# pengzai6666/deequ

Hardware: AMD Instinct MI355X
Metric: rows/sec & HBM GB/s for analyzer-suite scan, 1B rows x 8 cols, 1/2/4/8 GPUs (higher is better)
Workload: dtype int64+f64; 1 GPU; C2: 1000000000 rows/GPU x 8 cols (4 int64 + 4 fp64), 65 scan-shareable analyzers (incl. 8 ApproxCountDistinct) fused in one pass; rows_per_gpu=1000000000, columns=8, analyzers=65, parallelism=dp1 (row shards, states all-gathered over RCCL)

## Files before the change

### deequ_amd/_lib.py

```python
from __future__ import annotations

import ctypes
import os
from ctypes import (POINTER, Structure, c_char_p, c_double, c_int, c_int32, c_int64, c_size_t,
                    c_uint8, c_uint64, c_void_p)

LIB_PATH = os.environ.get("DEEQU_AMD_LIB") or os.path.join(
    os.path.dirname(os.path.abspath(__file__)), "libdeequ_amd.so")

DQ_OK, DQ_ERR_INVALID, DQ_ERR_UNSUPPORTED, DQ_ERR_DEVICE, DQ_ERR_OOM, DQ_ERR_STATE, DQ_ERR_SPACE = range(7)

DQ_T_BOOL, DQ_T_INT8, DQ_T_INT16, DQ_T_INT32, DQ_T_INT64, DQ_T_FLOAT32, DQ_T_FLOAT64, DQ_T_UTF8 = range(1, 9)
DQ_T_DECIMAL128 = 9
DQ_COL_DEVICE = 0x1

(DQ_OP_SIZE, DQ_OP_COMPLETENESS, DQ_OP_COMPLIANCE, DQ_OP_SUM, DQ_OP_MEAN, DQ_OP_STDDEV,
 DQ_OP_MINIMUM, DQ_OP_MAXIMUM, DQ_OP_APPROX_COUNT_DISTINCT, DQ_OP_DATATYPE, DQ_OP_MIN_LENGTH,
 DQ_OP_MAX_LENGTH, DQ_OP_CORRELATION, DQ_OP_PATTERN_MATCH) = range(1, 15)

DQ_P_COLUMN, DQ_P_LIT_INT, DQ_P_LIT_FLOAT, DQ_P_LIT_NULL, DQ_P_COALESCE, DQ_P_LIT_STRING = 1, 2, 3, 4, 5, 6
DQ_P_CAST_DOUBLE = 7
DQ_P_CAST = 8
DQ_P_EQ, DQ_P_NE, DQ_P_LT, DQ_P_LE, DQ_P_GT, DQ_P_GE, DQ_P_EQ_NULLSAFE = 10, 11, 12, 13, 14, 15, 16
DQ_P_IS_NULL, DQ_P_IS_NOT_NULL = 20, 21
# ... 150 lines not shown
    "dq_diag_key_pack": (c_int, [c_char_p, c_int32, POINTER(c_uint64), c_char_p, POINTER(c_int32), POINTER(c_int32)]),
    "dq_diag_uuid_pack": (c_int, [c_char_p, c_int32, POINTER(c_uint64), c_char_p, POINTER(c_int32)]),
    "dq_diag_eval_predicate": (c_int, [POINTER(DqPredicate), POINTER(DqColumn), c_int, c_int64, c_void_p]),
    "dq_diag_regex_match": (c_int, [c_char_p, c_int32, c_char_p, c_int64, POINTER(c_int32), POINTER(c_int32),
                                    POINTER(c_int32)]),
    "dq_diag_regex_match_mode": (c_int, [c_char_p, c_int32, c_int32, c_char_p, c_int64, POINTER(c_int32),
                                         POINTER(c_int32), POINTER(c_int32), c_void_p, c_int64, POINTER(c_int64)]),
    "dq_diag_plan_match_tasks": (c_int, [c_void_p, POINTER(c_int32), POINTER(c_int32)]),
    "dq_diag_kll_sketch": (c_int, [c_void_p, c_void_p, c_int64, c_int32, c_double, c_int64, c_void_p, c_int64,
                                   POINTER(c_int64)]),
    "dq_diag_schema_cell": (c_int, [c_int32, c_char_p, c_int64, c_int32, c_int32, POINTER(c_int32),
                                    POINTER(c_int64)]),
    "dq_diag_decimal_to_double": (c_int, [c_uint64, c_int64, c_int32, POINTER(c_double), POINTER(c_int32)]),
    "dq_diag_decimal_bytes": (c_int, [c_uint64, c_int64, c_char_p, POINTER(c_int32)]),
    "dq_diag_plan_groups": (c_int, [c_void_p, POINTER(c_int64), c_int32, POINTER(c_int32), POINTER(c_int64)]),
}


SIGNATURES = {
    "dq_last_error": (c_char_p, []),
    "dq_abi_version": (c_int, []),
    "dq_device_count": (c_int, [POINTER(c_int)]),
    "dq_release_cached_memory": (c_int, [c_int]),
    "dq_ctx_create": (c_int, [c_int, c_int, POINTER(c_void_p)]),
    "dq_ctx_destroy": (c_int, [c_void_p]),
    "dq_plan_create": (c_int, [c_void_p, POINTER(DqOp), c_int, POINTER(c_int32), c_int, POINTER(c_void_p)]),
    "dq_plan_destroy": (c_int, [c_void_p]),
    "dq_plan_create_packed": (c_int, [c_void_p, c_char_p, c_size_t, POINTER(c_int32), c_int, POINTER(c_void_p)]),
    "dq_op_supported": (c_int, [POINTER(DqOp), POINTER(c_int32), c_int]),
    "dq_plan_consume": (c_int, [c_void_p, POINTER(DqColumn), c_int, c_int64]),
# ... 130 lines not shown
PLAN_LAUNCHES = ("regex", "string_pass", "hll", "datatype", "strlen", "corr", "dec")


def diag_plan_groups(plan_handle):
    n = ctypes.c_int32(0)
    launches = (c_int64 * 10)()
    check(lib().dq_diag_plan_groups(plan_handle, None, 0, ctypes.byref(n), launches))
    groups = (c_int64 * (6 * max(1, n.value)))()
    check(lib().dq_diag_plan_groups(plan_handle, groups, n.value, ctypes.byref(n), launches))
    out = [tuple(groups[6 * g:6 * g + 6]) for g in range(n.value)]
    info = dict(zip(PLAN_LAUNCHES, launches[:7]))
    info.update(rows=launches[7], dec_per_cu=launches[8], n_cu=launches[9])
    return out, info


REGEX_MODES = {"find_non_empty": 0, "find": 1, "full": 2}


def diag_regex_match(pattern: bytes, text: bytes, mode: str = "find_non_empty", want_image: bool = False):
    m, ns, nc = c_int32(0), c_int32(0), c_int32(0)
    size = c_int64(0)
    args = (pattern, len(pattern), REGEX_MODES[mode], text, len(text), ctypes.byref(m), ctypes.byref(ns), ctypes.byref(nc))
    check(lib().dq_diag_regex_match_mode(*args, None, 0, ctypes.byref(size)))
    if not want_image:
        return m.value, ns.value, nc.value
    buf = ctypes.create_string_buffer(size.value)
    check(lib().dq_diag_regex_match_mode(*args, buf, size.value, ctypes.byref(size)))
    return m.value, ns.value, nc.value, buf.raw


# ... 28 lines not shown
```

### deequ_amd/csrc/dq_api.cpp

```cpp
#include <algorithm>
#include <cmath>
#include <cstdio>
#include <cstdlib>
#include <cstring>
#include <deque>
#include <limits>
#include <memory>
#include <mutex>
#include <unordered_map>
#include <string>
#include <vector>

#include "dq_internal.h"
#include "dq_keypack.h"
#include "dq_uuidpack.h"
#include "dq_numparse.h"
#include "dq_decimal.h"
#include "dq_predeval.h"
#include "dq_regex.h"
#include "dq_kll.h"
#include "dq_quantile.h"
#include "dq_schema.h"
#include "../../include/deequ_amd_diag.h"
#include "hll_p9_tables.h"
// ... 822 lines not shown
  DevBuf d_tasks, d_groups, d_ranges, d_hll, d_progs, d_insns, d_pool, d_acc, d_partials, d_regs,
      d_cols, d_masks, d_mask_words, d_dtype, d_dtype_counts, d_len, d_len_out, d_corr, d_corr_part, d_corr_acc, d_str, d_rx, d_rx_dfas, d_rx_out,
      d_dec, d_dec_acc, d_dec_part, d_match, d_match_words;
  int64_t mask_words = 0;
  void* h_desc = nullptr;
  size_t h_desc_size = 0;
  void* h_back = nullptr;
  size_t h_back_size = 0;
  hipEvent_t desc_done = nullptr;
  bool desc_pending = false;
  int64_t total_rows = 0;
  int target_blocks = 2048;
  int n_cu = 0;
  int scan_rounds = 6;
  int max_blocks = 0;
  std::vector<int64_t> diag_group_bpt;
  int64_t diag_launch_bpt[7] = {0, 0, 0, 0, 0, 0, 0};
  int64_t diag_rows = 0;
  int64_t cap_blocks(int64_t bpt) const { return max_blocks > 0 ? std::min<int64_t>(bpt, max_blocks) : bpt; }
  uint64_t batch_seq = 0;
  hipEvent_t copy_done[2] = {nullptr, nullptr}, scan_done[2] = {nullptr, nullptr};
  hipStream_t side_stream = nullptr;
  hipEvent_t side_ready = nullptr, side_done = nullptr;

  ~dq_plan() {
    if (stream) {
      (void)hipStreamSynchronize(stream);
    }
    if (side_stream) (void)hipStreamSynchronize(side_stream);
    if (side_ready) (void)hipEventDestroy(side_ready);
// ... 453 lines not shown
                      std::max<size_t>(1, plan->scan_tasks.size()) * sizeof(PartRange);
  if (e == hipSuccess) e = PinnedPool::get().alloc(plan->h_desc_size, &plan->h_desc);
  if (e != hipSuccess) {
    delete plan;
    return fail(DQ_ERR_DEVICE, std::string("stream/event/pinned allocation failed: ") + hipGetErrorString(e));
  }
  plan->resize_stage(n_columns);
  hipDeviceProp_t prop;
  if (hipGetDeviceProperties(&prop, ctx->device) == hipSuccess)
  {
    plan->target_blocks = std::max(256, prop.multiProcessorCount * 8);
    plan->n_cu = prop.multiProcessorCount;
  }
  if (const char* r = std::getenv("DQ_SCAN_ROUNDS")) plan->scan_rounds = std::max(0, std::atoi(r));
  if (const char* r = std::getenv("DQ_SCAN_MAX_BLOCKS")) plan->max_blocks = std::max(0, std::atoi(r));
  if ((s = dq_plan_reset(plan)) != DQ_OK) {
    delete plan;
    return s;
  }
  *out = plan;
  return DQ_OK;
}

extern "C" dq_status dq_plan_destroy(dq_plan* plan) {
  delete plan;
  return DQ_OK;
}

extern "C" dq_status dq_diag_plan_groups(dq_plan* plan, int64_t* groups, int32_t capacity, int32_t* n_groups,
                                         int64_t* launches) {
// ... 3 lines not shown
  const bool ran = plan->diag_group_bpt.size() == plan->groups.size() && plan->diag_rows > 0;
  for (size_t g = 0; g < plan->groups.size() && (int32_t)g < capacity; ++g) {
    const ScanGroup& G = plan->groups[g];
    int64_t* o = groups + 6 * g;
    o[0] = G.kind;
    o[1] = G.kind == 0 ? 0 : G.ptype;
    o[2] = G.np;
    o[3] = (int64_t)G.tasks.size();
    o[4] = ran ? plan->diag_group_bpt[g] : 0;
    o[5] = plan->group_per_cu.size() == plan->groups.size() ? plan->group_per_cu[g] : 0;
  }
  for (int k = 0; k < 7; ++k) launches[k] = ran ? plan->diag_launch_bpt[k] : 0;
  launches[7] = ran ? plan->diag_rows : 0;
  launches[8] = plan->dec_per_cu > 0 ? plan->dec_per_cu : 0;
  launches[9] = plan->n_cu;
  return DQ_OK;
}

extern "C" void* dq_plan_stream(dq_plan* plan) { return plan ? (void*)plan->stream : nullptr; }

extern "C" dq_status dq_plan_op_status(dq_plan* plan, int op) {
  if (!plan) return fail(DQ_ERR_INVALID, "plan is NULL");
  if (op < 0 || op >= (int)plan->slots.size()) return fail(DQ_ERR_INVALID, "op index out of range");
  if (plan->op_status.size() != plan->slots.size()) return fail(DQ_ERR_STATE, "dq_plan_finish has not run");
  if (plan->op_status[op] != DQ_OK && op < (int)plan->op_message.size() && !plan->op_message[op].empty())
    return fail(plan->op_status[op], plan->op_message[op]);
  if (plan->op_status[op] != DQ_OK)
    return fail(plan->op_status[op], "a string -> double cast in this op's predicate met a number off the exact "
                                     "fast path (> 19 significant digits, |exponent| > 22 or hex): route it to Spark");
  return DQ_OK;
// ... 197 lines not shown
                                                                 plan->groups[q].np);
      }
      const int per_cu = plan->group_per_cu[g];
      if (per_cu > 0) bpt = std::max<int64_t>(1, (int64_t)plan->n_cu * per_cu * plan->scan_rounds / ng);
    }
    bpt = plan->cap_blocks(std::max<int64_t>(1, std::min<int64_t>(bpt, chunks)));
    bpt = std::max<int64_t>(bpt, (chunks + (((int64_t)1 << 27) / kScanRowAlign) - 1) /
                                     (((int64_t)1 << 27) / kScanRowAlign));
    group_bpt[g] = bpt;
    group_base[g] = part_total;
    for (int64_t i = 0; i < ng; ++i)
      h_ranges[plan->groups[g].tasks[i]] = PartRange{part_total + i * bpt, (int32_t)bpt, 0};
    part_total += bpt * ng;
  }
  plan->diag_group_bpt = group_bpt;
  for (int64_t& b : plan->diag_launch_bpt) b = 0;
  plan->diag_rows = n_rows;
  if (n_scan > 0) DQ_TRY(plan->d_partials.ensure((size_t)part_total * sizeof(ScanAcc)));

  DQ_HIP(hipMemcpyAsync(plan->d_cols.ptr, h_cols, n_columns * sizeof(DevColumn), hipMemcpyHostToDevice, plan->stream));
  if (n_progs > 0)
    DQ_HIP(hipMemcpyAsync(plan->d_masks.ptr, h_masks, n_progs * sizeof(DevMask), hipMemcpyHostToDevice, plan->stream));
  if (n_scan > 0)
    DQ_HIP(hipMemcpyAsync(plan->d_ranges.ptr, h_ranges, n_scan * sizeof(PartRange), hipMemcpyHostToDevice, plan->stream));
  DQ_HIP(hipEventRecord(plan->desc_done, plan->stream));
  plan->desc_pending = true;

  const DevColumn* d_cols = static_cast<const DevColumn*>(plan->d_cols.ptr);
  const DevMask* d_masks = static_cast<const DevMask*>(plan->d_masks.ptr);
  const int n_match = (int)plan->match_tasks.size();
// ... 32 lines not shown
    hipStream_t ss = side ? plan->side_stream : plan->stream;
    int64_t bpt = std::max<int64_t>(1, plan->target_blocks / n_str);
    bpt = plan->cap_blocks(std::min<int64_t>(bpt, chunks));
    plan->diag_launch_bpt[1] = bpt;
    DQ_HIP(launch_string_pass(static_cast<const StrTask*>(plan->d_str.ptr), n_str, d_cols, d_masks, n_rows, (int)bpt,
                              static_cast<uint32_t*>(plan->d_regs.ptr),
                              static_cast<unsigned long long*>(plan->d_dtype_counts.ptr), ss));
    if (side) DQ_HIP(hipEventRecord(plan->side_done, ss));
  }
  if (n_scan > 0) {
    ScanAcc* parts = static_cast<ScanAcc*>(plan->d_partials.ptr);
    const ScanTask* d_tasks = static_cast<const ScanTask*>(plan->d_tasks.ptr);
    const int32_t* d_groups = static_cast<const int32_t*>(plan->d_groups.ptr);
    for (size_t g = 0; g < plan->groups.size(); ++g) {
      const ScanGroup& G = plan->groups[g];
      if (G.kind == 2)
        DQ_HIP(launch_scan_fast(G.ptype, G.np, d_tasks, d_groups + G.dev_offset, (int)G.tasks.size(), d_cols, n_rows,
                                (int)group_bpt[g], parts + group_base[g], static_cast<uint32_t*>(plan->d_regs.ptr),
                                plan->stream));
      else
        DQ_HIP(launch_scan_group(G.kind, G.ptype, G.np, d_tasks, d_groups + G.dev_offset, (int)G.tasks.size(),
                                 d_cols, d_masks, n_rows, (int)group_bpt[g], parts + group_base[g],
                                 static_cast<uint32_t*>(plan->d_regs.ptr), plan->stream));
    }
    DQ_HIP(launch_scan_reduce(parts, static_cast<const PartRange*>(plan->d_ranges.ptr), n_scan,
                              static_cast<ScanAcc*>(plan->d_acc.ptr), plan->stream));
  }
  const int n_hll = (int)plan->hll_launch.size();
  if (n_hll > 0) {
    int64_t bpt = std::max<int64_t>(1, plan->target_blocks / n_hll);
    bpt = plan->cap_blocks(std::min<int64_t>(bpt, chunks));
    plan->diag_launch_bpt[2] = bpt;
    DQ_HIP(launch_hll(static_cast<const HllTask*>(plan->d_hll.ptr), n_hll, d_cols, d_masks, n_rows, (int)bpt,
                      static_cast<uint32_t*>(plan->d_regs.ptr), plan->stream));
  }
// ... 948 lines not shown
```

### deequ_amd/csrc/dq_internal.h

```cpp
#pragma once

#include <hip/hip_runtime.h>
#include <stdint.h>

#include "../../include/deequ_amd.h"

namespace dq {

constexpr int kBlock = 256;
constexpr int kMaxPreds = 8;
constexpr int kMaxStack = 8;
constexpr int kHllM = 512;
constexpr int kHllIdxShift = 55;
constexpr uint64_t kHllWPadding = 1ull << 8;
constexpr int kScanRowAlign = 2048;

struct DevColumn {
  const uint8_t* validity;
  const void* values;
  const int32_t* offsets;
  int32_t type;
  int32_t pad;
};

// ... 365 lines not shown
                                  unsigned long long big_cap, uint32_t* d_smax, int write_all, hipStream_t stream,
                                  const FreqCompact* compact = nullptr);
hipError_t launch_freq_expand(const FreqTable& T, const FreqCompact& cmp, hipStream_t stream);
hipError_t launch_freq_export_compact(const FreqCompact& cmp, uint64_t n_slices, unsigned long long min_count,
                                      const FreqOut& out, const uint32_t* d_smax, hipStream_t stream);
hipError_t launch_freq_rehash(const FreqSlot* d_old, uint64_t old_n, const FreqTable& T, hipStream_t stream);

hipError_t launch_scan_group(int kind, int ptype, int np, const ScanTask* d_tasks,
                             const int32_t* d_group, int n_group, const DevColumn* d_cols,
                             const DevMask* d_masks, int64_t n_rows, int blocks_per_task,
                             ScanAcc* d_partials, uint32_t* d_hll_regs, hipStream_t stream);
constexpr int FAST_STATS = 8;
constexpr int FAST_HLL = 16;
hipError_t launch_scan_fast(int ptype, int variant, const ScanTask* d_tasks, const int32_t* d_group, int n_group,
                            const DevColumn* d_cols, int64_t n_rows, int blocks_per_task, ScanAcc* d_partials,
                            uint32_t* d_hll_regs, hipStream_t stream);
int scan_fast_blocks_per_cu(int ptype, int variant);
hipError_t launch_diag_hash(int blocks, int iters, bool with_hll, uint64_t* sink, hipStream_t s);
int scan_group_blocks_per_cu(int kind, int ptype, int np);
hipError_t launch_scan_reduce(const ScanAcc* d_partials, const PartRange* d_ranges, int n_tasks,
                              ScanAcc* d_acc, hipStream_t stream);
hipError_t launch_string_pass(const StrTask* d_tasks, int n_tasks, const DevColumn* d_cols, const DevMask* d_masks,
                              int64_t n_rows, int blocks_per_task, uint32_t* d_registers, unsigned long long* d_counts,
                              hipStream_t stream);
hipError_t launch_hll(const HllTask* d_tasks, int n_tasks, const DevColumn* d_cols,
                      const DevMask* d_masks, int64_t n_rows, int blocks_per_task,
                      uint32_t* d_registers, hipStream_t stream);
hipError_t launch_predicates(const PredProgram* d_progs, int n_progs, const PredInsn* d_insns,
                             const uint8_t* d_pool, const DevColumn* d_cols, int64_t n_rows,
                             uint64_t* d_mask_words, int64_t words_per_mask, bool with_cast, hipStream_t stream,
                             const uint64_t* d_match_words = nullptr);
hipError_t launch_match_mask(const MatchTask* d_tasks, int n_tasks, const DevColumn* d_cols, const uint8_t* d_dfas,
// ... 186 lines not shown
```

### deequ_amd/csrc/dq_scan_fast.hip

```cpp
#include "dq_scan_common.h"

namespace dq {

namespace {

enum FastPK : int { PK_NONE = 0, PK_LT_I = 1, PK_EQ_I = 2, PK_LT_F = 3, PK_EQ_F = 4 };

constexpr uint32_t kRankMarker = 0xFFFFFFFFu;

__device__ inline uint32_t sel32(uint32_t x, uint32_t m, uint32_t c) {
  uint32_t r;
  asm("v_bitop3_b32 %0, %1, %2, %3 bitop3:0xe2" : "=v"(r) : "v"(x), "v"(m), "v"(c));
  return r;
}

__device__ inline double i64_to_f64(uint32_t lo, uint32_t hi) {
  return fma((double)(int32_t)hi, 0x1p32, (double)lo);
}

__device__ inline double uniform_f64(double v) {
  const uint64_t b = __builtin_bit_cast(uint64_t, v);
  const uint32_t lo = __builtin_amdgcn_readfirstlane((uint32_t)b), hi = __builtin_amdgcn_readfirstlane((uint32_t)(b >> 32));
  return __builtin_bit_cast(double, ((uint64_t)hi << 32) | lo);
}
// ... 128 lines not shown
  }
}

typedef uint32_t v4u __attribute__((ext_vector_type(4)));

#ifndef DQ_FAST_UNROLL
#define DQ_FAST_UNROLL 4
#endif
#ifndef DQ_FAST_WAVES
#define DQ_FAST_WAVES 1
#endif
#ifndef DQ_VALID_AUX
#define DQ_VALID_AUX 0
#endif
constexpr int kFastUnroll = DQ_FAST_UNROLL;

constexpr int64_t kNtMinRows = (int64_t)1 << 24;
struct FastLoad {
  v4u vec[kFastUnroll];
  uint32_t vb[kFastUnroll];
};

__device__ inline void fast_load(FastLoad& L, __amdgpu_buffer_rsrc_t rv, __amdgpu_buffer_rsrc_t rvalid, uint32_t it,
                                 bool nt) {
  constexpr uint32_t ROWS_PER_ITER = (uint32_t)kBlock * 2 * kFastUnroll;
  const uint32_t tid = threadIdx.x;
#pragma unroll
  for (int u = 0; u < kFastUnroll; ++u) {
    const uint32_t r0 = it * ROWS_PER_ITER + ((uint32_t)u * kBlock + tid) * 2u;
    if (nt) {
// ... 99 lines not shown
    a.n_sel += bit;
    a.n_rows += 1;
    fast_row<T, PK, STATS, false, MEMBER, EXACT>(a, lo, hi, m, shift, cshift, dsum, lit_i, lit_f, lregs, false);
    if constexpr (__is_same(T, double) && STATS) {
      const double x = __builtin_bit_cast(double, ((uint64_t)hi << 32) | lo);
      if (bit && x != x) *s_nan = 1u;
    }
    if constexpr (HLL) {
      double unused = 0.0;
      fast_row<T, PK_NONE, false, true, MEMBER>(a, lo, hi, m, shift, cshift, unused, lit_i, lit_f, lregs, true);
    }
  }
  if constexpr (__is_same(T, double) && STATS) neumaier_add(a.fs, a.fc, dsum);
}

__device__ inline void fast_acc_init(FastAcc& a) {
  a.n_sel = a.n_rows = 0u;
  a.isum = 0u;
  a.s1 = a.s2 = 0.0;
  a.fs = a.fc = 0.0;
  a.fmin = __builtin_huge_val();
  a.fmax = -__builtin_huge_val();
  a.pc = 0u;
}

}

#ifdef DQ_SCAN_DIAG
__device__ unsigned long long g_scan_diag[4];
#define DQ_SCAN_COUNT(i) do { if (threadIdx.x == 0) atomicAdd(&g_scan_diag[i], 1ull); } while (0)
#else
#define DQ_SCAN_COUNT(i) do { } while (0)
#endif

template <typename T, int PK, bool STATS, bool HLL>
__global__ __launch_bounds__(kBlock) __attribute__((amdgpu_waves_per_eu(DQ_FAST_WAVES))) void dq_scan_fast_kernel(const ScanTask* __restrict__ tasks,
                                                              const int32_t* __restrict__ group,
                                                              const DevColumn* __restrict__ cols, int64_t n_rows,
                                                              ScanAcc* partials, uint32_t* __restrict__ hll_regs) {
  constexpr bool FP = __is_same(T, double);
  constexpr bool INT_STATS = !FP && STATS;
  const ScanTask& task = tasks[group[blockIdx.y]];
  int64_t row_begin, row_end;
  chunk_of_block(n_rows, row_begin, row_end);
  const bool nt = n_rows >= kNtMinRows;
  const uint32_t span = (uint32_t)(row_end - row_begin);
  __shared__ uint32_t lregs[kHllM];
  __shared__ uint32_t lflag[kHllM / 32];
  __shared__ uint32_t s_nan;
  if constexpr (HLL) {
    for (int r = threadIdx.x; r < kHllM; r += kBlock) lregs[r] = 0xFFFFFFFFu;
  }
  if (threadIdx.x == 0) s_nan = 0u;
  __syncthreads();
  const DevColumn& col = cols[task.primary];
  const __amdgpu_buffer_rsrc_t rv = make_rsrc(static_cast<const uint64_t*>(col.values) + row_begin, span * 8u);
  const bool has_valid = col.validity != nullptr;
  const uint32_t no_valid = has_valid ? 0u : 0xffu;
  const __amdgpu_buffer_rsrc_t rvalid =
      make_rsrc(has_valid ? col.validity + (row_begin >> 3) : nullptr, has_valid ? (span + 7u) >> 3 : 0u);
  int64_t lit_i = 0;
  double lit_f = 0.0;
  bool inv = false;
  if constexpr (PK != PK_NONE) {
    lit_i = task.preds[0].lit_i;
    lit_f = task.preds[0].lit_f;
    inv = (task.preds[0].cmp_sel & CS_INV) != 0;
  }

  const uint32_t lane = threadIdx.x & 63u;
  const uint32_t wave = threadIdx.x >> 6;
  uint32_t sh_lo = 0u, sh_hi = 0u;
  uint32_t any_lo = 0u, any_hi = 0u;
// ... 34 lines not shown
      member = true;
      break;
    }
  }
  sh_lo = __builtin_amdgcn_readfirstlane(sh_lo);
  sh_hi = __builtin_amdgcn_readfirstlane(sh_hi);
  const double shift = uniform_f64(FP ? __builtin_bit_cast(double, ((uint64_t)sh_hi << 32) | sh_lo)
                                      : i64_to_f64(sh_lo, sh_hi));
  const double cshift = uniform_f64(0x1.8p52 + shift);
  const double shift_any = FP ? shift : i64_to_f64(any_lo, any_hi);

  FastAcc a;
  fast_acc_init(a);
  constexpr uint32_t ROWS_PER_ITER = (uint32_t)kBlock * 2u * kFastUnroll;
  const uint32_t full_iters = span / ROWS_PER_ITER;
  if (member) {
    fast_main_loop<T, PK, STATS, HLL, true>(a, rv, rvalid, no_valid, full_iters, sh_lo, sh_hi, shift, cshift, lit_i,
                                            lit_f, lregs, &s_nan, nt);
    fast_tail<T, PK, STATS, HLL, true>(a, rv, rvalid, no_valid, full_iters * ROWS_PER_ITER, span, sh_lo, sh_hi,
                                       shift, cshift, lit_i, lit_f, lregs, &s_nan);
  } else {
    fast_main_loop<T, PK, STATS, HLL, false>(a, rv, rvalid, no_valid, full_iters, sh_lo, sh_hi, shift, cshift, lit_i,
                                             lit_f, lregs, &s_nan, nt);
    fast_tail<T, PK, STATS, HLL, false>(a, rv, rvalid, no_valid, full_iters * ROWS_PER_ITER, span, sh_lo, sh_hi,
                                        shift, cshift, lit_i, lit_f, lregs, &s_nan);
  }

  bool exact_stats = false;
  uint32_t mom_sel = a.n_sel;
  if constexpr (INT_STATS) {
    const double dmax = (a.fmin <= a.fmax) ? fmax(fabs(a.fmin), fabs(a.fmax)) : 0.0;
    const bool bad = a.n_rows > 0 && (dmax >= 0x1p50 || dmax * (double)a.n_rows >= 0x1p62 || a.s2 != a.s2);
    if (__syncthreads_or(bad)) {
      DQ_SCAN_COUNT(0);
      exact_stats = true;
      FastAcc e;
      fast_acc_init(e);
      if (found_any)
        fast_tail<T, PK_NONE, true, false, true, true>(e, rv, rvalid, no_valid, 0u, span, any_lo, any_hi, shift_any,
                                                       cshift, lit_i, lit_f, lregs, &s_nan);
      else
        fast_tail<T, PK_NONE, true, false, false, true>(e, rv, rvalid, no_valid, 0u, span, 0u, 0u, 0.0, cshift,
                                                        lit_i, lit_f, lregs, &s_nan);
      a.s1 = e.s1;
      a.s2 = e.s2;
      mom_sel = e.n_sel;
      a.fmin = e.fmin;
      a.fmax = e.fmax;
    } else {
      a.fmin = a.fmin + shift;
      a.fmax = a.fmax + shift;
      a.s1 = (double)(int64_t)(a.isum - (uint64_t)a.n_rows * (((uint64_t)sh_hi << 32) | sh_lo));
    }
  }

  const bool lane0 = lane == 0;
  double mom_shift = (INT_STATS && exact_stats) ? (found_any ? shift_any : 0.0) : shift;
  uint64_t mom_w = 0u;
  double S1 = 0.0, S2 = 0.0;
  if constexpr (STATS) {
    mom_w = wave_sum_u64(mom_sel);
    S1 = wave_sum_f64(a.s1);
    S2 = wave_sum_f64(a.s2);
    double wn = 0.0, wmean = 0.0;
    bool cancel = false;
    if (lane0 && mom_w > 0) {
      wn = (double)mom_w;
      wmean = mom_shift + S1 / wn;
      cancel = moments_cancel(wn, S1, S2);
    }
    if (__syncthreads_or(cancel)) {
      const double m = block_mean_of_waves(wn, wmean);
      if (fabs(m) < (FP ? 0x1p1000 : 0x1p62)) {
        uint32_t m_lo, m_hi;
        double m_shift;
        if constexpr (FP) {
          m_shift = m;
          const uint64_t b = __builtin_bit_cast(uint64_t, m);
// ... 50 lines not shown
        const uint32_t idx = h.hi >> 23;
        if (bit && ((lflag[idx >> 5] >> (idx & 31)) & 1u)) atomicMax(&lregs[idx], hll_rank_exact(h));
      }
      __syncthreads();
    }
    uint32_t* out = hll_regs + (int64_t)task.hll * kHllM;
    for (int r = threadIdx.x; r < kHllM; r += kBlock) {
      const uint32_t v = lregs[r];
      if (v) atomicMax(&out[r], v);
    }
  }
  __syncthreads();
  DQ_SCAN_COUNT(3);

  const uint64_t rows_w = wave_sum_u64(a.n_rows);
  const uint64_t sel_w = wave_sum_u64(a.n_sel);
  const uint64_t unsel_w = rows_w - sel_w;
  const uint64_t sh_bits = ((uint64_t)sh_hi << 32) | sh_lo;
  uint64_t isum = 0u;
  double mean = 0.0, m2 = 0.0, fs = 0.0, fc = 0.0;
  if constexpr (STATS) {
    isum = a.isum;
    fs = a.fs;
    fc = a.fc;
    if (lane0) {
      if constexpr (!FP) isum -= unsel_w * sh_bits;
      if (mom_w > 0) {
        const double n = (double)mom_w;
        mean = mom_shift + S1 / n;
        m2 = S2 - S1 * S1 / n;
        m2 = (m2 < 0.0) ? 0.0 : m2;
      }
      if constexpr (FP) {
        if (unsel_w > 0) {
          const double u = (double)unsel_w;
          const double p = u * shift;
          const double pe = (p - p == 0.0) ? fma(u, shift, -p) : 0.0;
          two_sum_merge(fs, fc, -p, -pe);
        }
      }
    }
  }
  uint64_t pm[1] = {0u}, pn[1] = {0u};
  if constexpr (PK != PK_NONE) {
    if (lane0) {
      bool pc_shift;
      if constexpr (PK == PK_LT_I) pc_shift = (int64_t)sh_bits < lit_i;
      else if constexpr (PK == PK_EQ_I) pc_shift = (int64_t)sh_bits == lit_i;
      else if constexpr (PK == PK_LT_F) pc_shift = shift < lit_f;
      else pc_shift = shift == lit_f;
      uint64_t c_all = inv ? rows_w - a.pc : a.pc;
      if (pc_shift != inv) c_all -= unsel_w;
      pm[0] = c_all;
      pn[0] = sel_w;
    }
  }
  const bool block_nan = FP && STATS && s_nan != 0u;
  block_reduce_store<1>(lane0 ? rows_w : 0u, lane0 ? rows_w : 0u, lane0 ? mom_w : 0u,
                        (threadIdx.x == 0 && block_nan) ? 1u : 0u, (int64_t)isum, INT64_MAX, INT64_MIN, fs, fc,
                        a.fmin, a.fmax, mean, m2, pm, pn, PK != PK_NONE ? 1 : 0,
                        &partials[(int64_t)blockIdx.y * gridDim.x + blockIdx.x]);
}

template <typename T, bool STATS, bool HLL>
static const void* fast_ptr(int pk) {
  switch (pk) {
    case PK_LT_I: return reinterpret_cast<const void*>(&dq_scan_fast_kernel<T, PK_LT_I, STATS, HLL>);
// ... 14 lines not shown
  return fast_ptr<T, false, false>(pk);
}

static const void* fast_kernel_for(int ptype, int variant) {
  if (ptype == DQ_T_INT64) return fast_kernel<int64_t>(variant);
  if (ptype == DQ_T_FLOAT64) {
    const int pk = variant & 7;
    if (pk == PK_LT_I || pk == PK_EQ_I) return nullptr;
    return fast_kernel<double>(variant);
  }
  return nullptr;
}

hipError_t launch_scan_fast(int ptype, int variant, const ScanTask* d_tasks, const int32_t* d_group, int n_group,
                            const DevColumn* d_cols, int64_t n_rows, int blocks_per_task, ScanAcc* d_partials,
                            uint32_t* d_hll_regs, hipStream_t stream) {
  if (n_group <= 0) return hipSuccess;
  const void* fn = fast_kernel_for(ptype, variant);
  if (!fn) return hipErrorInvalidValue;
  void* args[] = {&d_tasks, &d_group, &d_cols, &n_rows, &d_partials, &d_hll_regs};
#ifdef DQ_SCAN_DIAG
  {
    unsigned long long z[4] = {0, 0, 0, 0};
    (void)hipMemcpyToSymbolAsync(HIP_SYMBOL(g_scan_diag), z, sizeof(z), 0, hipMemcpyHostToDevice, stream);
    const hipError_t e = hipLaunchKernel(fn, dim3(blocks_per_task, n_group), dim3(kBlock), args, 0, stream);
    (void)hipMemcpyFromSymbolAsync(z, HIP_SYMBOL(g_scan_diag), sizeof(z), 0, hipMemcpyDeviceToHost, stream);
    (void)hipStreamSynchronize(stream);
    std::fprintf(stderr, "[scan_diag] rows %lld blocks %llu (x%d tasks): exact-int64 redo %llu, moment-guard redo %llu, "
                 "HLL marker re-rank %llu\n", (long long)n_rows, z[3], n_group, z[0], z[1], z[2]);
    return e;
  }
#endif
  return hipLaunchKernel(fn, dim3(blocks_per_task, n_group), dim3(kBlock), args, 0, stream);
}

// ... 10 lines not shown
```

### include/deequ_amd_diag.h

```cpp
#ifndef DEEQU_AMD_DIAG_H
#define DEEQU_AMD_DIAG_H

#include <stdint.h>
#include "deequ_amd.h"

#ifdef __cplusplus
extern "C" {
#endif

dq_status dq_diag_hash_rate(int device, int with_hll, int reps, double* hashes_per_sec);

dq_status dq_diag_freq_paths(dq_freq* f, int64_t* out);

dq_status dq_diag_freq_test_flags(dq_freq* f, int32_t flags);

dq_status dq_diag_parse_double(const uint8_t* s, int64_t n, double* out, int32_t* ok);

dq_status dq_diag_eval_predicate(const dq_predicate* p, const dq_column* columns, int n_columns, int64_t n_rows,
                                 uint8_t* out);

dq_status dq_diag_table_hash(int device, const uint64_t* k0, const uint64_t* k1, const uint32_t* len, int64_t n,
                             uint64_t* out);

dq_status dq_diag_key_pack(const uint8_t* key, int32_t len, uint64_t* packed, uint8_t* back, int32_t* back_len,
// ... 12 lines not shown

dq_status dq_diag_kll_sketch(const double* values, const uint8_t* valid, int64_t n, int32_t sketch_size,
                             double shrinking_factor, int64_t slab_rows, void* out, int64_t capacity,
                             int64_t* required);

dq_status dq_diag_schema_cell(int32_t kind, const uint8_t* text, int64_t n, int32_t precision, int32_t scale,
                              int32_t* result, int64_t* value);

dq_status dq_diag_decimal_to_double(uint64_t lo, int64_t hi, int32_t scale, double* out, int32_t* tier);

dq_status dq_diag_decimal_bytes(uint64_t lo, int64_t hi, uint8_t* out, int32_t* len);

dq_status dq_diag_plan_groups(dq_plan* plan, int64_t* groups, int32_t capacity, int32_t* n_groups,
                              int64_t* launches);

#ifdef __cplusplus
}
#endif

#endif
```

Measured before the change: 74.17 billion rows/s.

## Add lane-mask scan path using wave-level validity bitmasks for HLL groups

Adds a lane-mask variant of the fast scan kernel. Each wave loads 64-bit validity words through scalar loads, uses them as exec masks via inverse ballot, and counts selected rows with popcount, instead of having every lane load and shift validity bytes. HLL keys are batched and grouped before LDS min updates. The finish logic is adjusted for moments and predicate counts, since masked-off rows are no longer folded in as shift values. The path is on by default for HLL variants and needs 4-byte-aligned validity. It brings extra register pressure and new numeric paths for integer sums.

```diff
diff --git a/deequ_amd/_lib.py b/deequ_amd/_lib.py
--- a/deequ_amd/_lib.py
+++ b/deequ_amd/_lib.py
@@ -188,6 +188,7 @@
     "dq_diag_decimal_to_double": (c_int, [c_uint64, c_int64, c_int32, POINTER(c_double), POINTER(c_int32)]),
     "dq_diag_decimal_bytes": (c_int, [c_uint64, c_int64, c_char_p, POINTER(c_int32)]),
     "dq_diag_plan_groups": (c_int, [c_void_p, POINTER(c_int64), c_int32, POINTER(c_int32), POINTER(c_int64)]),
+    "dq_diag_plan_lanemask": (c_int, [c_void_p, POINTER(c_int32), c_int32, POINTER(c_int32)]),
 }
 
 
@@ -348,6 +349,14 @@
     return out, info
 
 
+def diag_plan_lanemask(plan_handle):
+    n = ctypes.c_int32(0)
+    check(lib().dq_diag_plan_lanemask(plan_handle, None, 0, ctypes.byref(n)))
+    tasks = (c_int32 * max(1, n.value))()
+    check(lib().dq_diag_plan_lanemask(plan_handle, tasks, n.value, ctypes.byref(n)))
+    return [bool(tasks[t]) for t in range(n.value)]
+
+
 REGEX_MODES = {"find_non_empty": 0, "find": 1, "full": 2}
 
 
diff --git a/deequ_amd/csrc/dq_api.cpp b/deequ_amd/csrc/dq_api.cpp
--- a/deequ_amd/csrc/dq_api.cpp
+++ b/deequ_amd/csrc/dq_api.cpp
@@ -860,6 +860,8 @@
   int n_cu = 0;
   int scan_rounds = 6;
   int max_blocks = 0;
+  int lanemask_mode = 1;
+  std::vector<int32_t> diag_task_lanemask;
   std::vector<int64_t> diag_group_bpt;
   int64_t diag_launch_bpt[7] = {0, 0, 0, 0, 0, 0, 0};
   int64_t diag_rows = 0;
@@ -1343,6 +1345,7 @@
   }
   if (const char* r = std::getenv("DQ_SCAN_ROUNDS")) plan->scan_rounds = std::max(0, std::atoi(r));
   if (const char* r = std::getenv("DQ_SCAN_MAX_BLOCKS")) plan->max_blocks = std::max(0, std::atoi(r));
+  if (const char* r = std::getenv("DQ_SCAN_LANEMASK")) plan->lanemask_mode = std::min(2, std::max(0, std::atoi(r)));
   if ((s = dq_plan_reset(plan)) != DQ_OK) {
     delete plan;
     return s;
@@ -1376,6 +1379,16 @@
   launches[7] = ran ? plan->diag_rows : 0;
   launches[8] = plan->dec_per_cu > 0 ? plan->dec_per_cu : 0;
   launches[9] = plan->n_cu;
+  return DQ_OK;
+}
+
+extern "C" dq_status dq_diag_plan_lanemask(dq_plan* plan, int32_t* tasks, int32_t capacity, int32_t* n_tasks) {
+  if (!plan || !n_tasks || capacity < 0 || (capacity > 0 && !tasks))
+    return fail(DQ_ERR_INVALID, "dq_diag_plan_lanemask: NULL argument");
+  *n_tasks = (int32_t)plan->scan_tasks.size();
+  const bool ran = plan->diag_task_lanemask.size() == plan->scan_tasks.size() && plan->diag_rows > 0;
+  for (size_t t = 0; t < plan->scan_tasks.size() && (int32_t)t < capacity; ++t)
+    tasks[t] = ran ? plan->diag_task_lanemask[t] : 0;
   return DQ_OK;
 }
 
@@ -1603,6 +1616,7 @@
     part_total += bpt * ng;
   }
   plan->diag_group_bpt = group_bpt;
+  plan->diag_task_lanemask.assign((size_t)n_scan, 0);
   for (int64_t& b : plan->diag_launch_bpt) b = 0;
   plan->diag_rows = n_rows;
   if (n_scan > 0) DQ_TRY(plan->d_partials.ensure((size_t)part_total * sizeof(ScanAcc)));
@@ -1665,11 +1679,14 @@
     const int32_t* d_groups = static_cast<const int32_t*>(plan->d_groups.ptr);
     for (size_t g = 0; g < plan->groups.size(); ++g) {
       const ScanGroup& G = plan->groups[g];
-      if (G.kind == 2)
+      if (G.kind == 2) {
+        const bool lanemask = scan_fast_lanemask_variant(plan->lanemask_mode, G.np);
+        for (int32_t t : G.tasks)
+          plan->diag_task_lanemask[t] = scan_fast_lanemask(lanemask, h_cols[plan->scan_tasks[t].primary].validity);
         DQ_HIP(launch_scan_fast(G.ptype, G.np, d_tasks, d_groups + G.dev_offset, (int)G.tasks.size(), d_cols, n_rows,
                                 (int)group_bpt[g], parts + group_base[g], static_cast<uint32_t*>(plan->d_regs.ptr),
-                                plan->stream));
-      else
+                                lanemask, plan->stream));
+      } else
         DQ_HIP(launch_scan_group(G.kind, G.ptype, G.np, d_tasks, d_groups + G.dev_offset, (int)G.tasks.size(),
                                  d_cols, d_masks, n_rows, (int)group_bpt[g], parts + group_base[g],
                                  static_cast<uint32_t*>(plan->d_regs.ptr), plan->stream));
diff --git a/deequ_amd/csrc/dq_internal.h b/deequ_amd/csrc/dq_internal.h
--- a/deequ_amd/csrc/dq_internal.h
+++ b/deequ_amd/csrc/dq_internal.h
@@ -403,8 +403,14 @@
 constexpr int FAST_HLL = 16;
 hipError_t launch_scan_fast(int ptype, int variant, const ScanTask* d_tasks, const int32_t* d_group, int n_group,
                             const DevColumn* d_cols, int64_t n_rows, int blocks_per_task, ScanAcc* d_partials,
-                            uint32_t* d_hll_regs, hipStream_t stream);
+                            uint32_t* d_hll_regs, bool lanemask, hipStream_t stream);
 int scan_fast_blocks_per_cu(int ptype, int variant);
+__host__ __device__ inline bool scan_fast_lanemask(bool lanemask, const uint8_t* validity) {
+  return lanemask && (reinterpret_cast<uintptr_t>(validity) & 3u) == 0u;
+}
+inline bool scan_fast_lanemask_variant(int mode, int variant) {
+  return mode >= 2 || (mode == 1 && (variant & FAST_HLL) != 0);
+}
 hipError_t launch_diag_hash(int blocks, int iters, bool with_hll, uint64_t* sink, hipStream_t s);
 int scan_group_blocks_per_cu(int kind, int ptype, int np);
 hipError_t launch_scan_reduce(const ScanAcc* d_partials, const PartRange* d_ranges, int n_tasks,
diff --git a/deequ_amd/csrc/dq_scan_fast.hip b/deequ_amd/csrc/dq_scan_fast.hip
--- a/deequ_amd/csrc/dq_scan_fast.hip
+++ b/deequ_amd/csrc/dq_scan_fast.hip
@@ -166,6 +166,10 @@
 #define DQ_VALID_AUX 0
 #endif
 constexpr int kFastUnroll = DQ_FAST_UNROLL;
+#ifndef DQ_LM_HASH_GROUP
+#define DQ_LM_HASH_GROUP 4
+#endif
+constexpr int kLmHashGroup = DQ_LM_HASH_GROUP;
 
 constexpr int64_t kNtMinRows = (int64_t)1 << 24;
 struct FastLoad {
@@ -295,6 +299,186 @@
   if constexpr (__is_same(T, double) && STATS) neumaier_add(a.fs, a.fc, dsum);
 }
 
+typedef uint32_t v2u __attribute__((ext_vector_type(2)));
+typedef uint32_t lm_words __attribute__((ext_vector_type(16), aligned(4)));
+constexpr int kLmRows = 8;
+
+struct LmLoad {
+  v2u v[kLmRows];
+};
+struct LmMasks {
+  uint64_t m[kLmRows];
+};
+
+template <int AUX>
+__device__ inline void lm_load_aux(LmLoad& L, __amdgpu_buffer_rsrc_t rv, uint32_t it) {
+  const uint32_t tid = threadIdx.x;
+  const uint32_t r0 = it * ((uint32_t)kBlock * kLmRows) + (tid >> 6) * (64u * kLmRows) + (tid & 63u);
+#pragma unroll
+  for (int u = 0; u < kLmRows; ++u)
+    L.v[u] = __builtin_amdgcn_raw_buffer_load_b64(rv, (int)((r0 + (uint32_t)u * 64u) * 8u), 0, AUX);
+}
+__device__ inline void lm_load(LmLoad& L, __amdgpu_buffer_rsrc_t rv, uint32_t it, bool nt) {
+  if (nt) lm_load_aux<2>(L, rv, it);
+  else lm_load_aux<0>(L, rv, it);
+}
+
+__device__ inline void lm_load_masks(LmMasks& M, const uint8_t* vbase, uint32_t off) {
+  if (vbase) {
+    const lm_words w = *(const __attribute__((address_space(4))) lm_words*)(vbase + off);
+#pragma unroll
+    for (int u = 0; u < kLmRows; ++u) M.m[u] = ((uint64_t)w[2 * u + 1] << 32) | w[2 * u];
+  } else {
+#pragma unroll
+    for (int u = 0; u < kLmRows; ++u) M.m[u] = ~0ull;
+  }
+}
+
+template <typename T, int PK>
+__device__ inline bool fast_pred(uint32_t lo, uint32_t hi, int64_t lit_i, double lit_f) {
+  constexpr bool INT = !__is_same(T, double);
+  if constexpr (PK == PK_LT_I) return (int64_t)(((uint64_t)hi << 32) | lo) < lit_i;
+  else if constexpr (PK == PK_EQ_I) return (int64_t)(((uint64_t)hi << 32) | lo) == lit_i;
+  else {
+    const double xd = INT ? i64_to_f64(lo, hi) : __builtin_bit_cast(double, ((uint64_t)hi << 32) | lo);
+    if constexpr (PK == PK_LT_F) return xd < lit_f;
+    else return xd == lit_f;
+  }
+}
+
+template <typename T, int PK, bool STATS, bool HLL>
+__device__ inline void lm_compute(FastAcc& a, uint32_t& sel, const LmLoad& L, const uint8_t* vbase, uint32_t voff,
+                                  double shift, double cshift, int64_t lit_i, double lit_f, uint32_t* lregs,
+                                  uint32_t* s_nan) {
+  constexpr bool FP = __is_same(T, double);
+  constexpr int G = kLmHashGroup;
+  LmMasks M;
+  lm_load_masks(M, vbase, voff);
+  uint32_t koff[G], ks[G];
+  if constexpr (HLL) {
+#pragma unroll
+    for (int k = 0; k < G; ++k) hll_key_min(hash_halves<T>(L.v[k][0], L.v[k][1]), koff[k], ks[k]);
+    __builtin_amdgcn_sched_barrier(0);
+  }
+  double dsum = -0.0;
+#pragma unroll
+  for (int u = 0; u < kLmRows; ++u) {
+    sel += (uint32_t)__builtin_popcountll(M.m[u]);
+    if constexpr (PK != PK_NONE)
+      a.pc += __builtin_popcountll(__ballot(fast_pred<T, PK>(L.v[u][0], L.v[u][1], lit_i, lit_f)) & M.m[u]);
+  }
+#pragma unroll
+  for (int u = 0; u < kLmRows; ++u) {
+    if constexpr (STATS) {
+      if (__builtin_expect(__builtin_amdgcn_inverse_ballot_w64(M.m[u]), 1))
+        fast_row<T, PK_NONE, true, false, true>(a, L.v[u][0], L.v[u][1], ~0u, shift, cshift, dsum, lit_i, lit_f, lregs,
+                                                false);
+    }
+  }
+  bool nan_possible = false;
+  if constexpr (FP && !STATS && HLL) {
+    bool any = false;
+#pragma unroll
+    for (int u = 0; u < kLmRows; ++u) {
+      const double x = __builtin_bit_cast(double, ((uint64_t)L.v[u][1] << 32) | L.v[u][0]);
+      any = any || (x != x);
+    }
+    nan_possible = __ballot(any) != 0;
+  }
+  if constexpr (FP && STATS) {
+    nan_possible = __ballot(dsum != dsum) != 0;
+    if (nan_possible) {
+#pragma unroll
+      for (int u = 0; u < kLmRows; ++u) {
+        const double x = __builtin_bit_cast(double, ((uint64_t)L.v[u][1] << 32) | L.v[u][0]);
+        if (((M.m[u] >> (threadIdx.x & 63u)) & 1u) && is_nan_rare(x)) *s_nan = 1u;
+      }
+    }
+    neumaier_add(a.fs, a.fc, dsum);
+  }
+  if constexpr (HLL) {
+#pragma unroll
+    for (int g = 0; g < kLmRows; g += G) {
+      if (FP && nan_possible) {
+#pragma unroll
+        for (int k = 0; k < G; ++k) {
+          uint32_t hlo = L.v[g + k][0], hhi = L.v[g + k][1];
+          if (is_nan_rare(__builtin_bit_cast(double, ((uint64_t)hhi << 32) | hlo))) {
+            hlo = 0u;
+            hhi = 0x7ff80000u;
+          }
+          hll_key_min(hash_halves<T>(hlo, hhi), koff[k], ks[k]);
+        }
+      } else if (g > 0) {
+#pragma unroll
+        for (int k = 0; k < G; ++k) hll_key_min(hash_halves<T>(L.v[g + k][0], L.v[g + k][1]), koff[k], ks[k]);
+      }
+#pragma unroll
+      for (int k = 0; k < G; ++k)
+        if (__builtin_expect(__builtin_amdgcn_inverse_ballot_w64(M.m[g + k]), 1)) lds_min(lregs, koff[k], ks[k]);
+    }
+  }
+}
+
+template <typename T, int PK, bool STATS, bool HLL>
+__device__ inline void lm_main_loop(FastAcc& a, uint32_t& sel, __amdgpu_buffer_rsrc_t rv, const uint8_t* vbase,
+                                    uint32_t full_iters, double shift, double cshift, int64_t lit_i, double lit_f,
+                                    uint32_t* lregs, uint32_t* s_nan, bool nt) {
+  LmLoad A, B;
+  constexpr uint32_t ITER_BYTES = (uint32_t)kBlock * kLmRows / 8u;
+  const uint32_t woff = __builtin_amdgcn_readfirstlane((threadIdx.x >> 6) * (8u * kLmRows));
+  uint32_t it = 0;
+  if (full_iters > 0) lm_load(A, rv, 0, nt);
+#pragma unroll 1
+  for (; it + 1 < full_iters; it += 2) {
+    lm_load(B, rv, it + 1, nt);
+    lm_compute<T, PK, STATS, HLL>(a, sel, A, vbase, it * ITER_BYTES + woff, shift, cshift, lit_i, lit_f, lregs, s_nan);
+    lm_load(A, rv, it + 2, nt);
+    lm_compute<T, PK, STATS, HLL>(a, sel, B, vbase, (it + 1) * ITER_BYTES + woff, shift, cshift, lit_i, lit_f, lregs,
+                                  s_nan);
+  }
+  if (it < full_iters)
+    lm_compute<T, PK, STATS, HLL>(a, sel, A, vbase, it * ITER_BYTES + woff, shift, cshift, lit_i, lit_f, lregs, s_nan);
+  a.n_rows += full_iters * kLmRows;
+}
+
+template <typename T, int PK, bool STATS, bool HLL>
+__device__ inline void lm_tail(FastAcc& a, __amdgpu_buffer_rsrc_t rv, __amdgpu_buffer_rsrc_t rvalid, uint32_t no_valid,
+                               uint32_t first, uint32_t span, double shift, double cshift, int64_t lit_i,
+                               double lit_f, uint32_t* lregs, uint32_t* s_nan) {
+  double dsum = 0.0;
+  for (uint32_t r = first + threadIdx.x; r < span; r += kBlock) {
+    const auto v = __builtin_amdgcn_raw_buffer_load_b64(rv, (int)(r * 8u), 0, 0);
+    const uint32_t bit = (((uint32_t)__builtin_amdgcn_raw_buffer_load_b8(rvalid, (int)(r >> 3), 0, 0) | no_valid) >>
+                          (r & 7u)) & 1u;
+    const uint32_t lo = (uint32_t)v[0], hi = (uint32_t)v[1];
+    a.n_sel += bit;
+    a.n_rows += 1;
+    if constexpr (PK != PK_NONE)
+      a.pc += __builtin_popcountll(__ballot(bit != 0u && fast_pred<T, PK>(lo, hi, lit_i, lit_f)));
+    if (bit) {
+      fast_row<T, PK_NONE, STATS, false, true>(a, lo, hi, ~0u, shift, cshift, dsum, lit_i, lit_f, lregs, false);
+      if constexpr (__is_same(T, double) && STATS) {
+        const double x = __builtin_bit_cast(double, ((uint64_t)hi << 32) | lo);
+        if (x != x) *s_nan = 1u;
+      }
+      if constexpr (HLL) {
+        double unused = 0.0;
+        fast_row<T, PK_NONE, false, true, true>(a, lo, hi, ~0u, shift, cshift, unused, lit_i, lit_f, lregs, true);
+      }
+    }
+  }
+  if constexpr (__is_same(T, double) && STATS) neumaier_add(a.fs, a.fc, dsum);
+}
+
+__device__ inline double lm_wave_sum_less(int64_t v, uint64_t n, int64_t c) {
+  const uint64_t lo = wave_sum_u64((uint64_t)v & 0xffffffffull);
+  const int64_t hi = (int64_t)wave_sum_u64((uint64_t)(v >> 32));
+  const __int128 t = (((__int128)hi) << 32) + (__int128)lo - (__int128)n * (__int128)c;
+  const int64_t th = (int64_t)(t >> 32);
+  return fma((double)th, 0x1p32, (double)(uint32_t)t);
+}
+
 __device__ inline void fast_acc_init(FastAcc& a) {
   a.n_sel = a.n_rows = 0u;
   a.isum = 0u;
@@ -318,7 +502,8 @@
 __global__ __launch_bounds__(kBlock) __attribute__((amdgpu_waves_per_eu(DQ_FAST_WAVES))) void dq_scan_fast_kernel(const ScanTask* __restrict__ tasks,
                                                               const int32_t* __restrict__ group,
                                                               const DevColumn* __restrict__ cols, int64_t n_rows,
-                                                              ScanAcc* partials, uint32_t* __restrict__ hll_regs) {
+                                                              ScanAcc* partials, uint32_t* __restrict__ hll_regs,
+                                                              uint32_t lanemask) {
   constexpr bool FP = __is_same(T, double);
   constexpr bool INT_STATS = !FP && STATS;
   const ScanTask& task = tasks[group[blockIdx.y]];
@@ -338,6 +523,7 @@
   const __amdgpu_buffer_rsrc_t rv = make_rsrc(static_cast<const uint64_t*>(col.values) + row_begin, span * 8u);
   const bool has_valid = col.validity != nullptr;
   const uint32_t no_valid = has_valid ? 0u : 0xffu;
+  const bool lm = scan_fast_lanemask(lanemask != 0u, col.validity);
   const __amdgpu_buffer_rsrc_t rvalid =
       make_rsrc(has_valid ? col.validity + (row_begin >> 3) : nullptr, has_valid ? (span + 7u) >> 3 : 0u);
   int64_t lit_i = 0;
@@ -402,7 +588,13 @@
   fast_acc_init(a);
   constexpr uint32_t ROWS_PER_ITER = (uint32_t)kBlock * 2u * kFastUnroll;
   const uint32_t full_iters = span / ROWS_PER_ITER;
-  if (member) {
+  uint32_t sel_main = 0u;
+  if (lm) {
+    lm_main_loop<T, PK, STATS, HLL>(a, sel_main, rv, has_valid ? col.validity + (row_begin >> 3) : nullptr, full_iters,
+                                    shift, cshift, lit_i, lit_f, lregs, &s_nan, nt);
+    lm_tail<T, PK, STATS, HLL>(a, rv, rvalid, no_valid, full_iters * ROWS_PER_ITER, span, shift, cshift, lit_i, lit_f,
+                               lregs, &s_nan);
+  } else if (member) {
     fast_main_loop<T, PK, STATS, HLL, true>(a, rv, rvalid, no_valid, full_iters, sh_lo, sh_hi, shift, cshift, lit_i,
                                             lit_f, lregs, &s_nan, nt);
     fast_tail<T, PK, STATS, HLL, true>(a, rv, rvalid, no_valid, full_iters * ROWS_PER_ITER, span, sh_lo, sh_hi,
@@ -418,7 +610,8 @@
   uint32_t mom_sel = a.n_sel;
   if constexpr (INT_STATS) {
     const double dmax = (a.fmin <= a.fmax) ? fmax(fabs(a.fmin), fabs(a.fmax)) : 0.0;
-    const bool bad = a.n_rows > 0 && (dmax >= 0x1p50 || dmax * (double)a.n_rows >= 0x1p62 || a.s2 != a.s2);
+    const bool bad = a.n_rows > 0 && (dmax >= 0x1p50 || (dmax + (lm ? 0x1p50 : 0.0)) * (double)a.n_rows >= 0x1p62 ||
+                                      a.s2 != a.s2);
     if (__syncthreads_or(bad)) {
       DQ_SCAN_COUNT(0);
       exact_stats = true;
@@ -438,9 +631,10 @@
     } else {
       a.fmin = a.fmin + shift;
       a.fmax = a.fmax + shift;
-      a.s1 = (double)(int64_t)(a.isum - (uint64_t)a.n_rows * (((uint64_t)sh_hi << 32) | sh_lo));
-    }
-  }
+      a.s1 = lm ? 0.0 : (double)(int64_t)(a.isum - (uint64_t)a.n_rows * (((uint64_t)sh_hi << 32) | sh_lo));
+    }
+  }
+  const uint64_t sel_lm = lm ? wave_sum_u64(a.n_sel) + sel_main : 0u;
 
   const bool lane0 = lane == 0;
   double mom_shift = (INT_STATS && exact_stats) ? (found_any ? shift_any : 0.0) : shift;
@@ -450,6 +644,11 @@
     mom_w = wave_sum_u64(mom_sel);
     S1 = wave_sum_f64(a.s1);
     S2 = wave_sum_f64(a.s2);
+    if (lm && !exact_stats) {
+      mom_w = sel_lm;
+      if constexpr (INT_STATS)
+        S1 = lm_wave_sum_less((int64_t)a.isum, sel_lm, (int64_t)(((uint64_t)sh_hi << 32) | sh_lo));
+    }
     double wn = 0.0, wmean = 0.0;
     bool cancel = false;
     if (lane0 && mom_w > 0) {
@@ -530,8 +729,8 @@
   DQ_SCAN_COUNT(3);
 
   const uint64_t rows_w = wave_sum_u64(a.n_rows);
-  const uint64_t sel_w = wave_sum_u64(a.n_sel);
-  const uint64_t unsel_w = rows_w - sel_w;
+  const uint64_t sel_w = lm ? sel_lm : wave_sum_u64(a.n_sel);
+  const uint64_t unsel_w = lm ? 0u : rows_w - sel_w;
   const uint64_t sh_bits = ((uint64_t)sh_hi << 32) | sh_lo;
   uint64_t isum = 0u;
   double mean = 0.0, m2 = 0.0, fs = 0.0, fc = 0.0;
@@ -540,7 +739,9 @@
     fs = a.fs;
     fc = a.fc;
     if (lane0) {
-      if constexpr (!FP) isum -= unsel_w * sh_bits;
+      if constexpr (!FP) {
+        if (!lm) isum -= unsel_w * sh_bits;
+      }
       if (mom_w > 0) {
         const double n = (double)mom_w;
         mean = mom_shift + S1 / n;
@@ -548,7 +749,7 @@
         m2 = (m2 < 0.0) ? 0.0 : m2;
       }
       if constexpr (FP) {
-        if (unsel_w > 0) {
+        if (!lm && unsel_w > 0) {
           const double u = (double)unsel_w;
           const double p = u * shift;
           const double pe = (p - p == 0.0) ? fma(u, shift, -p) : 0.0;
@@ -565,8 +766,13 @@
       else if constexpr (PK == PK_EQ_I) pc_shift = (int64_t)sh_bits == lit_i;
       else if constexpr (PK == PK_LT_F) pc_shift = shift < lit_f;
       else pc_shift = shift == lit_f;
-      uint64_t c_all = inv ? rows_w - a.pc : a.pc;
-      if (pc_shift != inv) c_all -= unsel_w;
+      uint64_t c_all;
+      if (lm) {
+        c_all = inv ? sel_w - a.pc : a.pc;
+      } else {
+        c_all = inv ? rows_w - a.pc : a.pc;
+        if (pc_shift != inv) c_all -= unsel_w;
+      }
       pm[0] = c_all;
       pn[0] = sel_w;
     }
@@ -611,11 +817,12 @@
 
 hipError_t launch_scan_fast(int ptype, int variant, const ScanTask* d_tasks, const int32_t* d_group, int n_group,
                             const DevColumn* d_cols, int64_t n_rows, int blocks_per_task, ScanAcc* d_partials,
-                            uint32_t* d_hll_regs, hipStream_t stream) {
+                            uint32_t* d_hll_regs, bool lanemask, hipStream_t stream) {
   if (n_group <= 0) return hipSuccess;
   const void* fn = fast_kernel_for(ptype, variant);
   if (!fn) return hipErrorInvalidValue;
-  void* args[] = {&d_tasks, &d_group, &d_cols, &n_rows, &d_partials, &d_hll_regs};
+  uint32_t lm_arg = lanemask ? 1u : 0u;
+  void* args[] = {&d_tasks, &d_group, &d_cols, &n_rows, &d_partials, &d_hll_regs, &lm_arg};
 #ifdef DQ_SCAN_DIAG
   {
     unsigned long long z[4] = {0, 0, 0, 0};
diff --git a/include/deequ_amd_diag.h b/include/deequ_amd_diag.h
--- a/include/deequ_amd_diag.h
+++ b/include/deequ_amd_diag.h
@@ -50,6 +50,8 @@
 dq_status dq_diag_plan_groups(dq_plan* plan, int64_t* groups, int32_t capacity, int32_t* n_groups,
                               int64_t* launches);
 
+dq_status dq_diag_plan_lanemask(dq_plan* plan, int32_t* tasks, int32_t capacity, int32_t* n_tasks);
+
 #ifdef __cplusplus
 }
 #endif
```

Result: faster. 77.35 billion rows/s, median of 6 (+4.3%).
